# braincorp/bc-gym-planning-env

Hardware: AMD Instinct MI355X
Metric: env-steps/sec at N=65536 RandomMiniEnv, 1/2/4/8 MI355X; % HBM roofline (higher is better)
Workload: dtype f64

## Files before the change

bc_gym_planning_env_amd/csrc/bcp_step.h:

```cpp
#pragma once

#include <hip/hip_runtime.h>

#include <cstddef>
#include <cstdint>
#include <type_traits>

#include "bcp_device.h"
#include "bcp_raster.h"
#include "bcp_coop.h"

using namespace bcp;

struct DevState {
    double *x, *y, *angle, *v, *w, *steer, *wheel, *min_dist;
    int32_t *target_idx, *cur_iter;
    uint8_t* collided;
    double *pose_seen, *state_seen;
    double *control_q, *pose_q, *state_q;
};

struct MapDesc {
    const uint32_t* bits;
    const uint32_t* tiles;
// ... 630 lines not shown
{
    if (delay <= 0) return;
    const int slot = (k - 1) % delay;
    double* cell = q + ((int64_t)slot * W) * n + i;
    if (k <= delay) {
#pragma unroll
        for (int c = 0; c < W; ++c) cell[c * n] = v[c];
        if (k > 1) {
#pragma unroll
            for (int c = 0; c < W; ++c) v[c] = q[c * n + i];
        }
    } else {
#pragma unroll
        for (int c = 0; c < W; ++c) {
            const double first = cell[c * n];
            cell[c * n] = v[c];
            v[c] = first;
        }
    }
}

template <int W>
__device__ __forceinline__ void fifo_peek(const double* __restrict__ q, int delay, int64_t n, int64_t i, int k, double (&peeked)[W])
{
    if (delay <= 0 || k <= 1) return;
    const double* cell = q + ((int64_t)(k > delay ? (k - 1) % delay : 0) * W) * n + i;
#pragma unroll
    for (int c = 0; c < W; ++c) peeked[c] = cell[c * n];
}

template <int W>
__device__ __forceinline__ void fifo_push(double* __restrict__ q, int delay, int64_t n, int64_t i, int k, double (&v)[W],
                                          const double (&peeked)[W])
{
    if (delay <= 0) return;
    double* cell = q + ((int64_t)((k - 1) % delay) * W) * n + i;
#pragma unroll
    for (int c = 0; c < W; ++c) {
        cell[c * n] = v[c];
        if (k > 1) v[c] = peeked[c];
    }
}

constexpr int kWavePerPoseFrom = 1;
#ifdef BCP_DIAG
constexpr int kDiagBlocks = 4096;
__device__ unsigned long long g_diag[kDiagBlocks * 16];
#define DIAG_STAMP(k) do { if (threadIdx.x == 0 && blockIdx.x < 512) g_diag[blockIdx.x * 16 + (k)] = __builtin_amdgcn_s_memtime(); } while (0)
#define DIAG_STAMP_W(w, k) do { if (threadIdx.x == (w) * 64 && blockIdx.x < kDiagBlocks) g_diag[blockIdx.x * 16 + (k)] = __builtin_amdgcn_s_memtime(); } while (0)
#define DIAG_MAX(k, v) do { if ((threadIdx.x & 63) == 0 && blockIdx.x < 2048) atomicMax(&g_diag[(2048 + blockIdx.x) * 16 + (k)], (unsigned long long)(v)); } while (0)
#define DIAG_NOW() __builtin_amdgcn_s_memtime()
#define DIAG_REAL_ENTRY() do { if ((threadIdx.x & 63) == 0 && blockIdx.x < 1024) atomicMax(&g_diag[(3072 + blockIdx.x) * 16 + 0], ~(unsigned long long)__builtin_amdgcn_s_memrealtime()); } while (0)
#define DIAG_REAL_EXIT() do { if ((threadIdx.x & 63) == 0 && blockIdx.x < 1024) atomicMax(&g_diag[(3072 + blockIdx.x) * 16 + 1], (unsigned long long)__builtin_amdgcn_s_memrealtime()); } while (0)
#define DIAG_STAMP_U(w, k) do { if (threadIdx.x == (w) * 64 && blockIdx.x < 2048) g_diag[(2048 + blockIdx.x) * 16 + (k)] = __builtin_amdgcn_s_memtime(); } while (0)
#define DIAG_WAIT_VMEM() asm volatile("s_waitcnt vmcnt(0)" ::: "memory")
#define DIAG_STAMP_WAVES(base) do { if ((threadIdx.x & 63) == 0 && blockIdx.x < 256) g_diag[((base) + blockIdx.x) * 16 + (threadIdx.x >> 6)] = __builtin_amdgcn_s_memtime(); } while (0)
#define DIAG_MAX_ALL(k, v) do { if (blockIdx.x < 2048) atomicMax(&g_diag[(2048 + blockIdx.x) * 16 + (k)], (unsigned long long)(v)); } while (0)
extern "C" int bcp_diag_read(unsigned long long* out)
{
    return (int)hipMemcpyFromSymbol(out, HIP_SYMBOL(g_diag), sizeof(g_diag));
}
extern "C" int bcp_diag_clear()
{
    void* p = nullptr;
    if (hipGetSymbolAddress(&p, HIP_SYMBOL(g_diag)) != hipSuccess) return -1;
    return (int)hipMemset(p, 0, sizeof(g_diag));
}

#else
#define DIAG_STAMP(k) do { } while (0)
#define DIAG_STAMP_W(w, k) do { } while (0)
#define DIAG_MAX(k, v) do { } while (0)
#define DIAG_NOW() 0ull
#define DIAG_REAL_ENTRY() do { } while (0)
#define DIAG_REAL_EXIT() do { } while (0)
#define DIAG_STAMP_U(w, k) do { } while (0)
#define DIAG_WAIT_VMEM() do { } while (0)
#define DIAG_STAMP_WAVES(base) do { } while (0)
#define DIAG_MAX_ALL(k, v) do { } while (0)
#endif


extern __shared__ uint32_t lds_dyn[];

struct CollisionLds {
    bool staged;
    LdsWords bits;
    LdsF64 qverts;
    VertLds scratch;
    LdsU32 cells;
};

__device__ __forceinline__ CollisionLds collision_lds_setup(const DevParams& P, const MapDesc& map, int tid)
{
    CollisionLds L;
    const int map_words = map.in_lds ? map.rows * map.wpr : 0;
    const LdsU32 lds = (LdsU32)lds_dyn;
    for (int k = tid; k < map_words; k += kBlock) lds[k] = map.bits[k];
    const int q_off = (map_words + 1) & ~1;
    __attribute__((address_space(3))) double* q = (__attribute__((address_space(3))) double*)(lds + q_off);
    for (int k = tid; k < 2 * P.n_verts; k += kBlock) q[k] = P.qverts[k >> 1][k & 1];
    L.staged = map.in_lds != 0;
    L.bits = lds;
    L.qverts = q;
    L.scratch.base = lds + q_off + 4 * P.n_verts + tid;
    L.scratch.stride = kBlock;
    L.cells = lds + q_off + 4 * P.n_verts + 2 * P.n_verts * kBlock;
    __syncthreads();
    return L;
}

static size_t collision_lds_bytes(int n_verts, int in_lds, int rows, int wpr)
{
    size_t words = in_lds ? (size_t)rows * wpr : 0;
    words = (words + 1) & ~(size_t)1;
    words += 4 * (size_t)n_verts;
    words += 2 * (size_t)n_verts * kBlock;
    words += kSparseLdsWords;
    return words * sizeof(uint32_t);
}

__device__ __forceinline__ bool collides_wave(const DevParams& P, const MapDesc& map, const CullDesc& cull,
                                              const CollisionLds& L, int exact_mode, int dense_threshold, bool wide,
                                              bool active, int64_t env, double x, double y, double th)
{
    double ox = map.ox, oy = map.oy;
    if (map.origins) {
        ox = map.origins[2 * env + 0];
// ... 39 lines not shown
            else
                verdict = wide ? coop_collides_sparse<true>(P, L.qverts, c_, s_, px_, py_, words, map.rows, map.cols, map.wpr, L.cells)
                               : coop_collides_sparse<false>(P, L.qverts, c_, s_, px_, py_, words, map.rows, map.cols, map.wpr, L.cells);
        }
        if (verdict != kSparseTooMany) {
            h = verdict == kSparseHit;
        } else if (L.staged) {
            h = coop_collides(P, vqx, vqy, c_, s_, px_, py_, L.bits, map.rows, map.cols, map.wpr, wide);
        } else {
            h = coop_collides(P, vqx, vqy, c_, s_, px_, py_, words, map.rows, map.cols, map.wpr, wide);
        }
        if (lane_id() == src) hit = h;
    }
    return hit;
}

struct Pending {
    double c, s;
    int32_t px, py;
    Robot r;
    Pose old;
    double min_dist;
    double z[3];
    int32_t target, iter, err, drawn;
    int32_t collided;
    int32_t env_lo, env_hi;
    int32_t geom;
    double popped_pose[3], popped_state[7];
};

struct InitAhead {
    double x, y, th, v, w, steer, wheel, min_dist;
    int32_t target, iter, collided;
};

template <typename SP>
__device__ __forceinline__ InitAhead fetch_init_ahead(SP S, int64_t k, bool tri)
{
    InitAhead p;
    p.x = as_global(S->init.x)[k];
    p.y = as_global(S->init.y)[k];
    p.th = as_global(S->init.angle)[k];
    p.v = as_global(S->init.v)[k];
    p.w = as_global(S->init.w)[k];
    p.steer = tri ? as_global(S->init.steer)[k] : 0.0;
    p.wheel = tri ? as_global(S->init.wheel)[k] : 0.0;
    p.min_dist = as_global(S->init.min_dist)[k];
    p.target = as_global(S->init.target_idx)[k];
    p.iter = as_global(S->init.cur_iter)[k];
    p.collided = (int32_t)as_global(S->init.collided)[k];
    return p;
}

struct ScoredFree {
    double rew, min_dist;
    int target;
};

struct ParkedPose {
    double c, s;
    int32_t px, py;
    int32_t env_lo, env_hi;
    int32_t geom;
    int32_t verdict;
    double spec_rew, spec_min;
    int32_t spec_target, spec_ok;
};

template <typename SP>
__device__ __forceinline__ int64_t slot_of(SP S, int64_t i, const Pending& q)
{
    return S->geom_of_env ? (int64_t)q.geom : i;
}

template <bool PLAIN, typename A, typename SP>
__device__ __forceinline__ int finalize_env_from(const A& a, SP S, int64_t i, Pending& q, bool hit, LdsF64 lds_path = nullptr,
                                             const PathWindow* free_window = nullptr, bool have_score = false,
                                             ScoredFree score = ScoredFree(), int known_len = -1, bool score_fits_hit = false,
                                             int64_t out_base = 0, RecRedo redo = RecRedo{0.0, -1, false})
{
    const DevParams& P = *(const DevParams*)&S->P;
    const int pose_delay = PLAIN ? 0 : P.pose_delay, state_delay = PLAIN ? 0 : P.state_delay;
    const bool pure_pursuit = !PLAIN && P.reward_provider == BCP_REWARD_PURE_PURSUIT;
    const bool tri = P.model == BCP_MODEL_TRICYCLE;
    const int64_t n = S->n;
    Robot& r = q.r;
    if (hit) {
        r.p = q.old;
        r.v = 0.0;
        r.w = 0.0;
    }
    int iter = q.iter + 1;
    bool collided = q.collided != 0 || hit;
    double min_dist = q.min_dist;
    int target = q.target;
    double seen[3] = {r.p.x, r.p.y, r.p.th};
    double seen_rs[7] = {r.p.x, r.p.y, r.p.th, r.v, r.w, r.steer, r.wheel};
    if (pose_delay) fifo_push<3>(S->st.pose_q, pose_delay, n, i, iter, seen, q.popped_pose);
    if (state_delay) fifo_push<7>(S->st.state_q, state_delay, n, i, iter, seen_rs, q.popped_state);

    double rew = 0.0;
    int m;
    bool goal;
    const int64_t g = slot_of(S, i, q);
    const double* pts = S->path.pts + (S->path.shared ? 0 : g * (int64_t)S->path.max_len * 5);
    m = known_len >= 0 ? known_len : (S->path.shared ? S->path.max_len : S->path.lens[g]);
    if (pure_pursuit) {
        if (have_score && !hit) {
            rew = score.rew;
            min_dist = score.min_dist;
            target = score.target;
        } else if (!ABLATED(a, kAblateNoReward)) {
            rew = reward_pure_pursuit(pts, m, seen[0], seen[1], collided, min_dist, target);
        }
        goal = hypot(pts[5 * (m - 1)] - seen[0], pts[5 * (m - 1) + 1] - seen[1]) < 1.0;
    } else {
        if (have_score && (!hit || score_fits_hit || (pose_delay && iter > 1))) {
            rew = score.rew;
            min_dist = score.min_dist;
            target = score.target;
        } else if (!ABLATED(a, kAblateNoReward)) {
            const PathWindow w =
                (free_window && !hit && !pose_delay) ? *free_window : path_window_of(P, S->path.shared != 0, S->path.bbox, S->path.index, g, seen[0], seen[1]);
            if (lds_path && S->path.shared)
                rew = reward_step(P, lds_path, w, m, seen[0], seen[1], seen[2], min_dist, target);
            else
                rew = reward_step<PLAIN ? 4 : 2>(P, pts, w, m, seen[0], seen[1], seen[2], min_dist, target);
        }
        goal = target > m - 1;
    }
    const bool timeout = iter >= P.iteration_timeout;
    const bool done = goal || timeout || collided;

    const int64_t o = out_base + i;
    as_global(a.reward)[o] = rew;
    as_global(a.done)[o] = (uint8_t)done;
    if (a.collided_now) as_global(a.collided_now)[o] = (uint8_t)hit;
    if (a.err) as_global(a.err)[o] = q.err;
    if (a.noise_z_out) {
        const double nan = __builtin_nan("");
        as_global(a.noise_z_out)[3 * o + 0] = (q.drawn & 1) ? q.z[0] : nan;
        as_global(a.noise_z_out)[3 * o + 1] = (q.drawn & 2) ? q.z[1] : nan;
        as_global(a.noise_z_out)[3 * o + 2] = (q.drawn & 4) ? q.z[2] : nan;
    }

    const bool reset = done && (a.flags & BCP_STEP_AUTO_RESET);
    InitAhead ahead = InitAhead();
    if (reset) {
        int64_t k = i;
        if (S->geom_of_env) {
            k = S->next_geom ? as_global(S->next_geom)[g] : g;
            as_global(S->geom_of_env)[i] = (int32_t)k;
        }
        ahead = fetch_init_ahead(S, k, tri);
    }
    int rec_slot = -1;
    if (a.flags & kStepRecord) {
        const EpisodeRec& R = a.S->rec;
        double ret_sum = 0.0;
        if (R.ret) ret_sum = (redo.on ? redo.ret_before : as_global(R.ret)[i]) + rew;
        as_global(R.reason)[i] = done ? (uint8_t)((goal ? BCP_DONE_GOAL : 0) | (timeout ? BCP_DONE_TIMEOUT : 0) |
                                                  (collided ? BCP_DONE_COLLIDED : 0))
                                      : (uint8_t)0;
        const bool keeps = redo.on && redo.slot >= 0;
        const bool take = done && !keeps;
        const uint64_t takers = __ballot(take);
        if (takers) {
            const int first = (int)__ffsll((unsigned long long)takers) - 1;
            const int lane = lane_id();
            int base = 0;
            if (lane == first) base = (int)atomicAdd(R.work, (uint32_t)__popcll(takers));
            base = bcast_i(base, first);
            if (take) rec_slot = base + (int)__popcll(takers & ((1ull << lane) - 1ull));
        }
        if (keeps) rec_slot = redo.slot;
        if (done && rec_slot < R.capacity) {
            const int64_t j = rec_slot, c = R.capacity;
            as_global(R.env_id)[j] = (int32_t)i;
            as_global(R.geom)[j] = S->geom_of_env ? (int32_t)g : -1;
            if (R.ret) as_global(R.final_ret)[j] = ret_sum;
            as_global(R.fin.x)[j] = r.p.x;
            as_global(R.fin.y)[j] = r.p.y;
            as_global(R.fin.angle)[j] = r.p.th;
            as_global(R.fin.v)[j] = r.v;
            as_global(R.fin.w)[j] = r.w;
            if (tri) {
                as_global(R.fin.steer)[j] = r.steer;
                as_global(R.fin.wheel)[j] = r.wheel;
            }
            as_global(R.fin.min_dist)[j] = min_dist;
            as_global(R.fin.target_idx)[j] = target;
            as_global(R.fin.cur_iter)[j] = iter;
            as_global(R.fin.collided)[j] = (uint8_t)collided;
            if (pose_delay) {
#pragma unroll
                for (int k = 0; k < 3; ++k) R.fin.pose_seen[k * c + j] = seen[k];
            }
            if (state_delay) {
#pragma unroll
                for (int k = 0; k < 7; ++k) R.fin.state_seen[k * c + j] = seen_rs[k];
            }
        }
        if (!done) rec_slot = -1;
        if (R.ret) as_global(R.ret)[i] = reset ? 0.0 : ret_sum;
    }
    if (reset) {
        r.p.x = ahead.x;
// ... 355 lines not shown
                Pending q = *e;
                finalize_env<PLAIN>(a, i, q, true, nullptr, nullptr, false, ScoredFree(), -1, false,
                                    redo_of(a, (int64_t)idx * kShards + shard));
            }
        }
        if (a.flags & kStepRecord) {
            __syncthreads();
            if (threadIdx.x == 0) record_publish(a.S, gridDim.x);
        }
        return;
    }
    for (int idx = blockIdx.x / kShards; idx < a.hot.pending_cap; idx += stride) {
        const Pending* e = slots + (int64_t)idx * kShards;
        const double c = e->c, s = e->s;
        const int px = e->px, py = e->py;
        const int64_t i = ((int64_t)e->env_hi << 32) | (uint32_t)e->env_lo;
        const int64_t g = a.hot.geom_of_env ? (int64_t)e->geom : i;
        if (idx >= count) break;
        DIAG_STAMP(1);
        const uint32_t* words = a.hot.map_bits + (a.hot.map_shared ? 0 : g * a.hot.map_env_stride);
        bool hit = false;
        DIAG_STAMP(2);
        if (!ABLATED(a, kAblateNoCoop))
            hit = coop_collides_quad<WIDE>(P, vqx, vqy, c, s, px, py, words, a.hot.map_rows, a.hot.map_cols, a.hot.map_wpr, wave,
                                           (LdsU32)lds_dyn);
        DIAG_STAMP(3);
        hit = __syncthreads_or(hit);
        DIAG_STAMP(4);
        if (hit && threadIdx.x == 0) {
            Pending q = *e;
            finalize_env<PLAIN>(a, i, q, true, nullptr, nullptr, false, ScoredFree(), -1, false,
                                redo_of(a, (int64_t)idx * kShards + shard));
        }
    }
    if (a.flags & kStepRecord) {
        __syncthreads();
        if (threadIdx.x == 0) record_publish(a.S, gridDim.x);
    }
}


constexpr int kLocalPairsMax = 4;
constexpr int kLocalPairsDefault = 4;

typedef const __attribute__((address_space(4))) StepArgs& KernArgs;

constexpr int kScanItems = 1024;
constexpr int kHandDoubles = 8;
constexpr int kLocalMapWords = 4096;

typedef uint32_t u32x4 __attribute__((ext_vector_type(4)));
constexpr int kStaticChunks = (int)((offsetof(StepStatic, rec) + 15) / 16);

static size_t local_step_lds_bytes(int n_verts, int lds_path_doubles, int staged_map_words, bool plain = true, int pairs = kLocalPairsMax)
{
    const int kLocalPairs = pairs, kLocalWaves = 4 * pairs, kLocalEnvs = pairs * kBlock;
    size_t bytes = ((size_t)2 * n_verts + lds_path_doubles + (size_t)kLocalPairs * kHandDoubles * kBlock + 8) * sizeof(double);
    bytes += 2 * kBlock * sizeof(uint32_t);
    bytes += 16 * sizeof(int32_t);
    bytes = (bytes + 15) & ~(size_t)15;
    bytes += (size_t)kLocalEnvs * sizeof(ParkedPose);
    bytes += (size_t)kLocalWaves * kSparseLdsWords * sizeof(uint32_t);
    bytes += (size_t)staged_map_words * sizeof(uint32_t);
    bytes = (bytes + 15) & ~(size_t)15;
    bytes += kStaticChunks * 16;
    if (!plain) bytes += (size_t)10 * kLocalEnvs * sizeof(double);
    return bytes;
}

template <int NW>
__device__ __forceinline__ void fetch_words(const __attribute__((address_space(4))) void* p, uint32_t (&w)[NW])
{
    const __attribute__((address_space(4))) uint32_t* src = (const __attribute__((address_space(4))) uint32_t*)p;
#pragma unroll
    for (int k = 0; k < NW; ++k) w[k] = src[k];
}

template <int NW>
__device__ __forceinline__ void pin_words(uint32_t (&w)[NW])
{
#pragma unroll
    for (int k = 0; k < NW; ++k) {
        asm("" : "+s"(w[k]));
        w[k] = (uint32_t)__builtin_amdgcn_readfirstlane((int)w[k]);
    }
}

struct PrologueArgs {
    StepHot hot;
    const StepStatic* S;
    const void* actions;
    const double* noise_z;
    uint64_t* tick;
    uint32_t flags;
};

__device__ __forceinline__ uint64_t uniform_u64(uint64_t v)
{
    const uint32_t lo = (uint32_t)__builtin_amdgcn_readfirstlane((int)(uint32_t)v);
    const uint32_t hi = (uint32_t)__builtin_amdgcn_readfirstlane((int)(uint32_t)(v >> 32));
    return ((uint64_t)hi << 32) | lo;
}

static_assert(kStaticChunks <= 128, "*S is staged by the last two waves of a workgroup");
constexpr int kPollLimit = 1 << 16;
#define BOUNDED_POLL(cond, expired) do { int trips_ = 0; while (cond) { __builtin_amdgcn_s_sleep(1); if (++trips_ > kPollLimit) { (expired) = true; break; } } } while (0)
constexpr uint32_t kDiagWithholdVerdicts = 1u << 23;

typedef const __attribute__((address_space(4))) StepArgs* KernArgPtr;

template <bool WIDE, bool PLAIN, int PAIRS, bool ROLL>
__device__ __forceinline__ void step_local_body(KernArgPtr kernarg, const int rs)
{
    static_assert(PAIRS == 1 || PAIRS == 2 || PAIRS == 4, "a workgroup holds 1, 2 or 4 (mover, scorer, helper, helper) quartets");
    constexpr int kLocalPairs = PAIRS, kLocalWaves = 4 * PAIRS, kLocalEnvs = PAIRS * kBlock;
    constexpr int kPairShift = PAIRS == 4 ? 2 : (PAIRS == 2 ? 1 : 0);
    constexpr int kStaticFrom = (kLocalWaves - 2) * kBlock;
    constexpr int kCtlFrom = (kLocalWaves - 1) * kBlock;
    [[maybe_unused]] constexpr int kWScorer = PAIRS, kWHelper1 = 2 * PAIRS, kWHelper2 = 3 * PAIRS;
    DIAG_STAMP_WAVES(512);
    DIAG_REAL_ENTRY();
    const int tid = threadIdx.x, lane = tid & 63, wave = tid >> 6;
    const bool mover = wave < kLocalPairs, scorer = wave >= kLocalPairs && wave < 2 * kLocalPairs;
    const int pair = wave & (kLocalPairs - 1);
    KernArgs a = *kernarg;
    PrologueArgs L;
    {
        constexpr int kStateWords = PLAIN ? kHotStateWords : (int)(sizeof(DevState) / 4);
        uint32_t w_st[kStateWords], w_hot[kHotPrologueWords];
        fetch_words(&a.hot.st, w_st);
        fetch_words(&a.hot.n, w_hot);
        pin_words(w_st);
        pin_words(w_hot);
        __builtin_memset(&L.hot, 0, sizeof(L.hot));
        __builtin_memcpy(&L.hot.st, w_st, sizeof(w_st));
        __builtin_memcpy(&L.hot.n, w_hot, sizeof(w_hot));
        L.actions = L.hot.io_actions;
        L.noise_z = L.hot.io_noise_z;
        L.tick = L.hot.io_tick;
        L.flags = L.hot.io_flags;
        L.S = a.S;
        if (ROLL) {
            const int64_t row = (int64_t)rs * L.hot.n;
            L.actions = (const char*)L.actions + row * ((L.flags & BCP_STEP_ACTIONS_F32) ? 8 : 16);
            L.noise_z = L.noise_z ? L.noise_z + 3 * row : nullptr;
        }
    }
    const int64_t out_base = ROLL ? (int64_t)rs * L.hot.n : 0;
    const int hot_n_verts = L.hot.n_verts, hot_npath = L.hot.lds_path_doubles, hot_path_shared = L.hot.path_shared;
    const int hot_map_rows = L.hot.map_rows, hot_map_cols = L.hot.map_cols, hot_map_wpr = L.hot.map_wpr;
    const int hot_map_shared = L.hot.map_shared, hot_noise_on = L.hot.noise_on, hot_max_len = L.hot.path_max_len;
    const int64_t hot_n = L.hot.n;
    const bool scanner = PLAIN ? !mover : scorer;
    const int member = (wave >> kPairShift) - 1;

    __attribute__((address_space(3))) double* qv = (__attribute__((address_space(3))) double*)lds_dyn;
    const int nq = 2 * hot_n_verts;
    const int npath = hot_npath;
    const LdsF64 lds_path = npath ? (LdsF64)(qv + nq) : (LdsF64) nullptr;
    __attribute__((address_space(3))) double* hand_pose = qv + nq + npath + pair * kHandDoubles * kBlock;
    __attribute__((address_space(3))) double* hand_score = hand_pose + 3 * kBlock;
    __attribute__((address_space(3))) double* hand_heading = hand_pose + 6 * kBlock;
    __attribute__((address_space(3))) double* lds_box = qv + nq + npath + kLocalPairs * kHandDoubles * kBlock;
    __attribute__((address_space(3))) uint32_t* lds_index = (__attribute__((address_space(3))) uint32_t*)(lds_box + 8);
    __attribute__((address_space(3))) int32_t* ctl = (__attribute__((address_space(3))) int32_t*)(lds_index + 2 * kBlock);
    const uint32_t rec_off = (uint32_t)((((size_t)(nq + npath + kLocalPairs * kHandDoubles * kBlock + 8) * sizeof(double) +
                                          2 * kBlock * sizeof(uint32_t) + 16 * sizeof(int32_t)) + 15) & ~(size_t)15);
    __attribute__((address_space(3))) ParkedPose* rec =
        (__attribute__((address_space(3))) ParkedPose*)((__attribute__((address_space(3))) char*)lds_dyn + rec_off);
    const LdsU32 cell_list = (LdsU32)(rec + kLocalEnvs) + wave * kSparseLdsWords;
    const LdsU32 lds_map = (LdsU32)(rec + kLocalEnvs) + kLocalWaves * kSparseLdsWords;
    const int map_words = ((hot_map_shared != 0) & (hot_map_rows * hot_map_wpr <= kLocalMapWords)) ? hot_map_rows * hot_map_wpr : 0;
    const uint32_t static_off = (uint32_t)(((size_t)((__attribute__((address_space(3))) char*)(lds_map + map_words) -
                                                     (__attribute__((address_space(3))) char*)lds_dyn) + 15) & ~(size_t)15);
    __attribute__((address_space(3))) u32x4* lds_static = (__attribute__((address_space(3))) u32x4*)((__attribute__((address_space(3))) char*)lds_dyn + static_off);
    const __attribute__((address_space(3))) StepStatic* SL = (const __attribute__((address_space(3))) StepStatic*)lds_static;
    __attribute__((address_space(3))) double* fifo_stash = (__attribute__((address_space(3))) double*)(lds_static + kStaticChunks) + pair * kBlock + lane;

    DIAG_STAMP(0);
    DIAG_STAMP_WAVES(768);
    const int64_t gi = (int64_t)blockIdx.x * kLocalEnvs + pair * kBlock + lane;
    const bool active = gi < hot_n;
    const int64_t i = active ? gi : hot_n - 1;
    const bool noise_by_waves = (hot_noise_on != 0) & (L.noise_z == nullptr);

    uint64_t tick_counter = 0, tick_seed = 0;
    if (!mover) {
        int zero;
        asm("v_mov_b32 %0, 0" : "=v"(zero));
        const GlobalPtr<const uint64_t> t = as_global((const uint64_t*)L.tick) + zero;
        tick_counter = t[0];
        tick_seed = t[2];
    }
    Pending q;
    double cmd0 = 0.0, cmd1 = 0.0;
    float box[8] = {0, 0, 0, 0, 0, 0, 0, 0};
    float quant_inv = 0.0f;
    double old_angle = 0.0;
    double own_org_x = 0.0, own_org_y = 0.0;
    uint64_t own_len_shift = 0;
    const bool own_origin = !hot_path_shared || L.hot.map_origins != nullptr;
    if (mover) {
        load_env<PLAIN>(L, 0, 0, i, active, q, cmd0, cmd1, false);
        if (!hot_path_shared) {
            const int64_t g = L.hot.geom_of_env ? (int64_t)q.geom : i;
            own_org_x = as_global(L.hot.path_bbox)[g * kBoxDoubles + kBoxOrigin];
            own_org_y = as_global(L.hot.path_bbox)[g * kBoxDoubles + kBoxOrigin + 1];
            own_len_shift = as_global(reinterpret_cast<const uint64_t*>(L.hot.path_bbox))[g * kBoxDoubles + kBoxLenWord / 2];
        } else if (L.hot.map_origins) {
            const int64_t g = L.hot.geom_of_env ? (int64_t)q.geom : i;
            own_org_x = as_global(L.hot.map_origins)[2 * g + 0];
            own_org_y = as_global(L.hot.map_origins)[2 * g + 1];
        }
    } else {
        if (scanner) {
            if (!PLAIN) q.min_dist = as_global(L.hot.st.min_dist)[i];
            q.target = as_global(L.hot.st.target_idx)[i];
            q.geom = L.hot.geom_of_env ? as_global(L.hot.geom_of_env)[i] : 0;
            q.collided = PLAIN ? 0 : (int32_t)(as_global(L.hot.st.collided)[i] != 0);
            if (!hot_path_shared) {
                const int64_t g = L.hot.geom_of_env ? (int64_t)q.geom : i;
#pragma unroll
                for (int k = 0; k < 8; ++k) box[k] = as_global(reinterpret_cast<const float*>(L.hot.path_bbox + g * kBoxDoubles))[k];
                quant_inv = as_global(reinterpret_cast<const float*>(L.hot.path_bbox + g * kBoxDoubles))[kBoxQuantStep + 1];
                own_len_shift = as_global(reinterpret_cast<const uint64_t*>(L.hot.path_bbox))[g * kBoxDoubles + kBoxLenWord / 2];
            }
        }
        if (member == 1) old_angle = as_global(L.hot.st.angle)[i];
    }
    double rc[9] = {0, 0, 0, 0, 0, 0, 0, 0, 0};
    if (PLAIN && mover) {
// ... 57 lines not shown
    }
    if (tid >= kCtlFrom && tid < kCtlFrom + 16) ctl[tid - kCtlFrom] = 0;
    if (first_trip && tid >= kStaticFrom && tid < kStaticFrom + kStaticChunks) lds_static[tid - kStaticFrom] = st_static;
    DIAG_STAMP_WAVES(1024);
    __syncthreads();
    const DevParams& P = *(const DevParams*)&SL->P;
    const int map_rows = hot_map_rows, map_cols = hot_map_cols;
    const int my_len = hot_path_shared ? hot_max_len : (int)(uint32_t)own_len_shift;
    Pose new_pose;
    new_pose.x = new_pose.y = new_pose.th = 0.0;
    if (mover) {
        if (noise_by_waves) {
            q.z[0] = hand_score[lane];
            q.z[1] = hand_score[kBlock + lane];
            q.z[2] = hand_score[2 * kBlock + lane];
        }
        DIAG_STAMP(1);
        if (!PLAIN) drive = robot_step_begin(P, r, cmd0, cmd1);
        new_pose = robot_step_pose(P, r, drive, q.z, q.drawn);
        const bool delayed = !PLAIN && P.pose_delay > 0 && q.iter + 1 > 1;
        hand_pose[lane] = delayed ? fifo_stash[0] : new_pose.x;
        hand_pose[kBlock + lane] = delayed ? fifo_stash[kLocalEnvs] : new_pose.y;
        hand_pose[2 * kBlock + lane] = delayed ? fifo_stash[2 * kLocalEnvs] : new_pose.th;
        DIAG_STAMP(2);
    }
    if (!mover && member == 1) {
        double c0, s0;
        cos_sin(old_angle, c0, s0);
        hand_heading[lane] = c0;
        hand_heading[kBlock + lane] = s0;
        DIAG_STAMP_U(kWHelper1, 2);
    }
    if (!mover && first_trip) {
        constexpr int kStagers = (kLocalWaves - kLocalPairs) * kBlock;
        constexpr int kMapPerStager = (kLocalMapWords + kStagers - 1) / kStagers;
        constexpr int kBoxAt = kStagers >= 448 ? 256 : kStagers - 8;
        constexpr int kIndexAt = kStagers >= 448 ? 320 : kStagers - 136;
        const int nm = tid - kLocalPairs * kBlock;
        double st_q = 0.0, st_path = 0.0;
        float st_box = 0.0f;
        uint32_t st_index = 0;
        uint32_t st_map[kMapPerStager] = {};
        if (nm < nq) st_q = as_global(L.hot.qverts)[nm];
        if (nm < npath) st_path = as_global(L.hot.path_pts)[nm];
        if (hot_path_shared) {
            if (nm >= kBoxAt && nm < kBoxAt + 8) st_box = as_global(reinterpret_cast<const float*>(L.hot.path_bbox))[nm - kBoxAt];
            if (nm >= kIndexAt && nm < kIndexAt + 128) st_index = as_global(reinterpret_cast<const uint32_t*>(L.hot.path_index))[nm - kIndexAt];
        }
#pragma unroll
        for (int u = 0; u < kMapPerStager; ++u) {
            const int k = u * kStagers + nm;
            if (k < map_words) st_map[u] = as_global(L.hot.map_bits)[k];
        }
        if (nm < nq) qv[nm] = st_q;
        if (nm < npath) qv[nq + nm] = st_path;
        for (int k = kStagers + nm; k < npath; k += kStagers) qv[nq + k] = as_global(L.hot.path_pts)[k];
        if (hot_path_shared) {
            if (nm >= kBoxAt && nm < kBoxAt + 8) lds_box[nm - kBoxAt] = (double)st_box;
            if (nm >= kIndexAt && nm < kIndexAt + 128) lds_index[nm - kIndexAt] = st_index;
        }
#pragma unroll
        for (int u = 0; u < kMapPerStager; ++u) {
            const int k = u * kStagers + nm;
            if (k < map_words) lds_map[k] = st_map[u];
        }
    }
    DIAG_STAMP_WAVES(1536);
    __syncthreads();
    DIAG_STAMP(3);
    if (mover) {
        KnownHeading old_heading;
        old_heading.c0 = hand_heading[lane];
        old_heading.s0 = hand_heading[kBlock + lane];
        old_heading.known = true;
        q.err = robot_step_measure(P, r, new_pose, old_heading);
    }
    bool park = false;
    bool poll_expired = false;
    if (mover) {
        OuterParams outer = outer_params(*(const CullDesc*)&SL->cull);
        outer.near_tx = SL->cull.step_near_tx;
        outer.near_shift = SL->cull.step_near_shift;
        const double map_inv_res = SL->map.inv_res;
        const int64_t near_stride = SL->cull.step_near_stride;
        const double org_x = own_origin ? own_org_x : SL->map.ox, org_y = own_origin ? own_org_y : SL->map.oy;
        const int64_t g = slot_of(SL, i, q);
        const int px = (int)rint((r.p.x - org_x) * map_inv_res);
        const int py = (int)rint((r.p.y - org_y) * map_inv_res);
        double c, s;
        cos_sin(r.p.th, c, s);
        DIAG_STAMP_U(0, 4);
        const int64_t map_env = a.hot.map_shared ? 0 : g;
        int cls = kFree;
#ifdef BCP_DIAG
        if (!ABLATED(a, kAblateNoCollision | kAblateNoClassify))
#endif
        {
            if (a.hot.near) {
                cls = classify_near(outer, as_global(a.hot.near) + map_env * near_stride, map_rows, map_cols, px, py, c, s);
            } else {
                const OuterLookups look = outer_lookups_issue(*(const CullDesc*)&SL->cull, map_env, map_rows, map_cols, px, py, c, s);
                cls = outer_lookups_verdict(*(const CullDesc*)&SL->cull, look);
            }
        }
        if (!active) cls = kFree;
        DIAG_STAMP_U(0, 5);
        if (cls == kAmbiguous && !ABLATED(a, kAblateNoPark)) {
            park = true;
            q.c = c;
            q.s = s;
            q.px = px;
            q.py = py;
            q.env_lo = (int32_t)(uint32_t)i;
            q.env_hi = (int32_t)(i >> 32);
        }
    } else if (scanner && !ABLATED(a, kAblateNoReward)) {
        const double x = hand_pose[lane], y = hand_pose[kBlock + lane], th = hand_pose[2 * kBlock + lane];
// ... 179 lines not shown
    DIAG_STAMP_W(kWHelper1, 9);
    const double vqx = lane < P.n_verts ? qv[2 * lane] : 0.0, vqy = lane < P.n_verts ? qv[2 * lane + 1] : 0.0;
    DIAG_STAMP(7);
    __attribute__((address_space(3))) int* const ticket_word =
        lane == 0 ? (__attribute__((address_space(3))) int*)&ctl[1] : (__attribute__((address_space(3))) int*)(cell_list + lane);
    int ticket = __builtin_amdgcn_readfirstlane(__hip_atomic_fetch_add(ticket_word, lane == 0 ? 1 : 0, __ATOMIC_RELAXED, __HIP_MEMORY_SCOPE_WORKGROUP));
    while (ticket < n_parked) {
        DIAG_STAMP_W(kWHelper1, 10);
        __attribute__((address_space(3))) ParkedPose* e = rec + ticket;
        const double c = e->c, s = e->s;
        const int px = e->px, py = e->py;
        const int64_t env = ((int64_t)e->env_hi << 32) | (uint32_t)e->env_lo;
        const int64_t g = a.hot.map_shared ? 0 : (a.hot.geom_of_env ? (int64_t)e->geom : env);
        const uint32_t* words = a.hot.map_bits + g * a.hot.map_env_stride;
        const uint32_t* tiles = a.map_tiles + g * map_tile_words(a.hot.map_rows, a.hot.map_wpr);
        bool h = false;
        [[maybe_unused]] const unsigned long long test_from = DIAG_NOW();
        [[maybe_unused]] int how = 0;
        if (!ABLATED(a, kAblateNoCoop)) {
#ifdef BCP_DIAG
            unsigned long long phase[3] = {test_from, test_from, 0};
            unsigned long long* const phases = phase;
#else
            unsigned long long* const phases = nullptr;
#endif
            const int verdict = map_words
                ? coop_collides_sparse<WIDE>(P, (LdsF64)qv, c, s, px, py, (LdsWords)lds_map, a.hot.map_rows, a.hot.map_cols,
                                             a.hot.map_wpr, cell_list, phases)
                : coop_collides_sparse<WIDE, true>(P, (LdsF64)qv, c, s, px, py, as_global(tiles), a.hot.map_rows, a.hot.map_cols,
                                                   a.hot.map_wpr, cell_list, phases);
#ifdef BCP_DIAG
            if (threadIdx.x == kWHelper1 * 64 && blockIdx.x < 2048) {
                const unsigned long long now = DIAG_NOW();
                g_diag[(2048 + blockIdx.x) * 16 + 13] = ((phase[0] - test_from) << 40) | ((phase[1] - phase[0]) << 20) | (now - phase[1]);
                g_diag[(2048 + blockIdx.x) * 16 + 15] = phase[2];
            }
#endif
            h = verdict == kSparseHit;
            if (verdict == kSparseTooMany)
                h = coop_collides<WIDE>(P, vqx, vqy, c, s, px, py, words, a.hot.map_rows, a.hot.map_cols, a.hot.map_wpr);
            how = verdict;
        }
        DIAG_MAX(0, ((DIAG_NOW() - test_from) << 4) | (unsigned)how);
        DIAG_STAMP_W(kWHelper1, 11);
        bool post = lane == 0;
#ifdef BCP_DIAG
        post = post && !(a.flags & kDiagWithholdVerdicts);
#endif
        if (post) __hip_atomic_store(&e->verdict, h ? 2 : 1, __ATOMIC_RELEASE, __HIP_MEMORY_SCOPE_WORKGROUP);
        ticket = __builtin_amdgcn_readfirstlane(__hip_atomic_fetch_add(ticket_word, lane == 0 ? 1 : 0, __ATOMIC_RELAXED, __HIP_MEMORY_SCOPE_WORKGROUP));
        DIAG_STAMP_W(kWHelper1, 12);
    }
    if (mover) {
        int verdict = park ? 0 : 1;
        {
            int trips = 0;
            while (__ballot(verdict == 0)) {
                if (verdict == 0) verdict = __hip_atomic_load(&my_rec->verdict, __ATOMIC_ACQUIRE, __HIP_MEMORY_SCOPE_WORKGROUP);
                __builtin_amdgcn_s_sleep(1);
                if (++trips > kPollLimit) {
                    poll_expired = true;
                    if (verdict == 0) {
                        verdict = 1;
                        q.err |= BCP_ERR_INTERNAL;
                    }
                    break;
                }
            }
        }
        const bool hit_score = PLAIN && lds_path && a.hot.path_shared && !ABLATED(a, kAblateNoReward);
        int last_hit = -1;
        if (hit_score) {
            uint64_t hits = __ballot(park && verdict == 2);
            while (hits) {
                const int src = (int)__ffsll((unsigned long long)hits) - 1;
                hits &= hits - 1;
                const double ox = bcast_d(q.old.x, src), oy = bcast_d(q.old.y, src), oth = bcast_d(q.old.th, src);
                const int tg = bcast_i(q.target, src);
                const PathWindow w = path_window(P, (LdsF64)lds_box, (const __attribute__((address_space(3))) int16_t*)lds_index, ox, oy);
                const int found = coop_last_reached(P, lds_path, w, my_len, tg, ox, oy, oth);
                if (lane == src) last_hit = found;
            }
        }
        if (active) {
            const bool hit_now = park && verdict == 2;
            bool fits = hit_score && hit_now;
            if (fits) {
                sc.min_dist = q.min_dist;
                sc.target = q.target;
                sc.rew = reward_from_last(P, lds_path, my_len, last_hit, q.old.x, q.old.y, sc.min_dist, sc.target);
            } else if (PLAIN && hit_now && my_rec->spec_ok) {
                sc.rew = my_rec->spec_rew;
                sc.min_dist = my_rec->spec_min;
                sc.target = my_rec->spec_target;
                fits = true;
            }
            if (!PLAIN) {
#pragma unroll
                for (int k = 0; k < 3; ++k) q.popped_pose[k] = fifo_stash[k * kLocalEnvs];
#pragma unroll
                for (int k = 0; k < 7; ++k) q.popped_state[k] = fifo_stash[(3 + k) * kLocalEnvs];
            }
            finalize_env_from<PLAIN>(a, SL, i, q, hit_now, lds_path, nullptr, !ABLATED(a, kAblateNoReward), sc, my_len, fits, out_base);
        }
        if ((a.flags & kStepRecord) && lane == 0 &&
            __hip_atomic_fetch_add(&ctl[3], 1, __ATOMIC_ACQ_REL, __HIP_MEMORY_SCOPE_WORKGROUP) == kLocalPairs - 1) {
            __threadfence();
            unsigned int* ticket = reinterpret_cast<unsigned int*>(a.tick + kTickLocalTicket);
            if (atomicAdd(ticket, 1u) == gridDim.x - 1) {
                *ticket = 0u;
                a.tick[0] = a.tick[0] + 1;
                record_store_count(a.S->rec);
            }
        }
    }
    DIAG_STAMP(13);
    DIAG_STAMP_W(kWHelper1, 14);
#ifdef BCP_DIAG
    if (tid == 0 && blockIdx.x < kDiagBlocks) g_diag[blockIdx.x * 16 + 15] = (unsigned long long)n_parked;
#endif
    if (poll_expired && lane == 0) atomicAdd(reinterpret_cast<unsigned long long*>(a.tick + 4), 1ull);
    DIAG_REAL_EXIT();
    if ((a.flags & kStepAdvances) && tid == (kLocalWaves - 1) * kBlock) {
        if (n_parked) a.parked_slots[blockIdx.x] += (uint64_t)n_parked;
        if ((!ROLL || rs == a.rollout_steps - 1) && !(a.flags & kStepRecord)) {
            const unsigned int ticket_drawn =
                __hip_atomic_fetch_add((GlobalPtr<unsigned int>)(a.tick + kTickLocalTicket), 1u, __ATOMIC_RELAXED, __HIP_MEMORY_SCOPE_AGENT);
            if (ticket_drawn == gridDim.x - 1) {
                *reinterpret_cast<unsigned int*>(a.tick + kTickLocalTicket) = 0u;
                a.tick[0] = step_counter + 1;
            }
        }
    }
}

template <bool WIDE, bool PLAIN, int PAIRS>
__device__ __attribute__((noinline)) void step_local_trip(uint64_t kernarg_bits, int rs)
{
    const uint32_t lo = (uint32_t)__builtin_amdgcn_readfirstlane((int)(uint32_t)kernarg_bits);
    const uint32_t hi = (uint32_t)__builtin_amdgcn_readfirstlane((int)(uint32_t)(kernarg_bits >> 32));
    step_local_body<WIDE, PLAIN, PAIRS, true>((KernArgPtr)(uintptr_t)(((uint64_t)hi << 32) | lo), __builtin_amdgcn_readfirstlane(rs));
}

template <bool WIDE, bool PLAIN, int PAIRS, bool ROLL = false>
__global__ void __attribute__((amdgpu_flat_work_group_size(4 * PAIRS * kBlock, 4 * PAIRS * kBlock), amdgpu_waves_per_eu(4)))
step_local_kernel(const StepArgs launch_args)
{
    KernArgPtr kernarg = (KernArgPtr)__builtin_amdgcn_kernarg_segment_ptr();
    if constexpr (!ROLL) {
        step_local_body<WIDE, PLAIN, PAIRS, false>(kernarg, 0);
    } else {
        const int n_steps = kernarg->rollout_steps;
        for (int rs = 0; rs < n_steps; ++rs) {
            step_local_trip<WIDE, PLAIN, PAIRS>((uint64_t)(uintptr_t)kernarg, rs);
            __syncthreads();
        }
    }
// ... 2 lines not shown
```

bc_gym_planning_env_amd/csrc/bcp_step_host.h:

```cpp
#pragma once

static bool step_is_plain(const bcp_handle* h)
{
    const bcp_params& p = h->params;
    return p.control_delay == 0 && p.pose_delay == 0 && p.state_delay == 0 && p.reward_provider == BCP_REWARD_CONTINUOUS;
}

static bool step_uses_deferral(const bcp_handle* h)
{
    return h->defer && h->cull.on && h->exact_mode == 0 && h->pending.get() != nullptr;
}

static int step_form(const bcp_handle* h)
{
    if (!step_uses_deferral(h)) return 0;
    if (h->dense_threshold < 0) return 1;
    return (h->fused && h->adaptive) ? 3 : 2;
}

static int upload_step_static(bcp_handle* h, hipStream_t s)
{
    StepStatic& S = h->host_static;
    S.P = h->dev;
    S.map = h->map;
// ... 92 lines not shown
        default: return BCP_LOCAL_FN(false, false);
    }
#undef BCP_LOCAL_FN
}

static int local_pairs(const bcp_handle* h)
{
    if (h->local_pairs == 1 || h->local_pairs == 2 || h->local_pairs == 4) return h->local_pairs;
    return kLocalPairsDefault;
}

static int launch_step(bcp_handle* h, const bcp_step_io* io, uint32_t flags, hipStream_t s, bool first_only = false,
                       int32_t rollout_steps = 1)
{
    if (h->static_dirty) BCP_TRY(upload_step_static(h, s));
    const StepStatic& S = h->host_static;
    const int form = step_form(h);
    const bool fused = form == 3;
    if (!fused && h->edt_lazy) BCP_TRY(ensure_fields(h, s));
    if ((form == 1 || form == 2) && (h->last_step_form == 0 || h->last_step_form == 3)) BCP_TRY(rearm_parking(h, s));
    h->last_step_form = form;
    StepArgs a;
    a.S = h->dev_static.get();
    a.hot = h->host_hot;
    a.actions = io->actions;
    a.noise_z = io->noise_z;
    a.noise_z_out = io->noise_z_out;
    a.reward = io->reward;
    a.done = io->done;
    a.collided_now = io->collided_now;
    a.err = io->err;
    a.flags = flags;
    if (h->have_rec) a.flags |= kStepRecord;
    a.seed = a.step_counter = 0;
    a.pending_count = a.pending_next = nullptr;
    a.threshold_now = nullptr;
    a.threshold_next = a.inplace_count = a.inplace_next = nullptr;
    const bool adapt = h->adaptive && h->adapt.get() && S.pending && S.dense_threshold >= 0;
    a.tick = h->tick.get();
    a.parked_slots = nullptr;
    a.map_tiles = S.map.tiles;
    a.rollout_steps = 1;
    a.pending_base = h->pending_count.get();
    a.adapt_base = adapt ? h->adapt.get() : nullptr;
    const int blocks = (int)((h->n + kBlock - 1) / kBlock);
    const int variant = (S.wide ? 2 : 0) | (step_is_plain(h) ? 1 : 0);
    if (fused) {
        const bool roll = rollout_steps > 1;
        const int pairs = roll ? 4 : local_pairs(h);
        a.rollout_steps = rollout_steps;
        const int64_t bitmap_words = (int64_t)S.map.rows * S.map.wpr;
        const size_t lds = local_step_lds_bytes(h->params.n_verts, S.lds_path_doubles,
                                                (S.map.shared && bitmap_words <= kLocalMapWords) ? (int)bitmap_words : 0,
                                                step_is_plain(h), pairs);
        a.flags |= kStepAdvances;
        a.hot.io_flags = a.flags;
        a.hot.io_actions = a.actions;
        a.hot.io_noise_z = a.noise_z;
        a.hot.io_tick = a.tick;
        const int envs_per_group = pairs * kBlock;
        const dim3 grid((unsigned)((h->n + envs_per_group - 1) / envs_per_group)), block(4 * pairs * kBlock);
        if (!h->parked_slots.get()) {
            HIP_TRY(h->parked_slots.reserve((size_t)((h->n + kBlock - 1) / kBlock)));
            HIP_TRY(hipMemsetAsync(h->parked_slots.get(), 0, h->parked_slots.capacity() * sizeof(uint64_t), s));
        }
        a.parked_slots = h->parked_slots.get();
        return launch_variant(h, local_step_fn(variant, pairs, roll), grid, block, lds, s, a);
    }
    if (rollout_steps > 1) return fail(BCP_E_STATE, "launch_step: only the single-launch step form takes several steps per launch");
    if (form == 0) {
        const size_t lds = collision_lds_bytes(h->params.n_verts, h->map.in_lds, h->map.rows, h->map.wpr);
        a.flags |= kStepAdvances;
        hipLaunchKernelGGL(step_kernel, dim3(blocks), dim3(kBlock), lds, s, a);
        return BCP_OK;
    }
    const size_t lds1 = ((size_t)h->params.n_verts * 2 + S.lds_path_doubles) * sizeof(double);
    const size_t lds2 = (size_t)2 * 4 * (S.wide ? 8 : 3) * 64 * sizeof(uint32_t);
    const int waves = 2048;
    const bool second = !first_only && S.dense_threshold >= 0;
    if (!second) a.flags |= kStepAdvances;
    const size_t lds1p = lds1 + ((size_t)6 * kBlock + 8) * sizeof(double) + 2 * kBlock * sizeof(uint32_t);
    const int rc = launch_variant(h, kFastPairFn[variant], dim3(blocks), dim3(2 * kBlock), lds1p, s, a);
    if (rc != BCP_OK || !second) return rc;
    return launch_variant(h, kPendingFn[variant], dim3(waves), dim3(kBlock * kPendingWaves), lds2, s, a);
}

#ifdef BCP_DIAG
constexpr uint32_t kCallerFlags = BCP_STEP_AUTO_RESET | BCP_STEP_ACTIONS_F32 | kAblateNoCollision | kAblateNoReward |
                                  kAblateNoCoop | kAblateNoPark | kAblateNoClassify | kDiagWithholdVerdicts;
#else
constexpr uint32_t kCallerFlags = BCP_STEP_AUTO_RESET | BCP_STEP_ACTIONS_F32;
#endif

static int check_step(bcp_handle* h, const bcp_step_io* io, uint32_t flags, const char* who)
{
    if (!h || !io) return fail(BCP_E_INVALID, "%s: null argument", who);
    if (flags & ~kCallerFlags) return fail(BCP_E_INVALID, "%s: undefined flag bits 0x%x", who, flags & ~kCallerFlags);
    if (!h->have_map || !h->have_path || !h->have_state)
        return fail(BCP_E_STATE, "%s: costmaps, paths and state must be set first", who);
    if ((flags & BCP_STEP_AUTO_RESET) && !h->have_init)
        return fail(BCP_E_STATE, "%s: BCP_STEP_AUTO_RESET needs bcp_bind_initial_state", who);
    if (!io->actions || !io->reward || !io->done) return fail(BCP_E_INVALID, "%s: actions/reward/done are required", who);
    return BCP_OK;
}

constexpr uint32_t kWatchdogSteps = 256;

// ... 282 lines not shown
```

Baseline: 5.802 billion.

## Overlap hit-rescoring with verdict polling and stage reset init state in LDS

Moves the cooperative last-reached path scan and reward rescoring for parked poses inside the verdict-polling loop, so the scoring runs while waves would otherwise sleep waiting for collision verdicts. Prefetches per-env reset init state into LDS during the staging phase for plain, non-geometry runs, so auto-reset reads LDS instead of scattered global loads in the tail. Packs the output pointers into a compact TailArgs fetched as words. This costs extra LDS per pair, which may reduce occupancy, and the staging loads run even for envs that never reset. It also adds diagnostic tail stamps that compile away by default.

```diff
diff --git a/bc_gym_planning_env_amd/csrc/bcp_step.h b/bc_gym_planning_env_amd/csrc/bcp_step.h
--- a/bc_gym_planning_env_amd/csrc/bcp_step.h
+++ b/bc_gym_planning_env_amd/csrc/bcp_step.h
@@ -706,6 +706,8 @@
 #define DIAG_NOW() __builtin_amdgcn_s_memtime()
 #define DIAG_REAL_ENTRY() do { if ((threadIdx.x & 63) == 0 && blockIdx.x < 1024) atomicMax(&g_diag[(3072 + blockIdx.x) * 16 + 0], ~(unsigned long long)__builtin_amdgcn_s_memrealtime()); } while (0)
 #define DIAG_REAL_EXIT() do { if ((threadIdx.x & 63) == 0 && blockIdx.x < 1024) atomicMax(&g_diag[(3072 + blockIdx.x) * 16 + 1], (unsigned long long)__builtin_amdgcn_s_memrealtime()); } while (0)
+#define DIAG_TAIL_MAX(k, v) do { if (blockIdx.x < 1024) atomicMax(&g_diag[(3072 + blockIdx.x) * 16 + (k)], (unsigned long long)(v)); } while (0)
+#define DIAG_TAIL_STAMP(k) do { if ((threadIdx.x & 63) == 0) DIAG_TAIL_MAX(k, __builtin_amdgcn_s_memtime()); } while (0)
 #define DIAG_STAMP_U(w, k) do { if (threadIdx.x == (w) * 64 && blockIdx.x < 2048) g_diag[(2048 + blockIdx.x) * 16 + (k)] = __builtin_amdgcn_s_memtime(); } while (0)
 #define DIAG_WAIT_VMEM() asm volatile("s_waitcnt vmcnt(0)" ::: "memory")
 #define DIAG_STAMP_WAVES(base) do { if ((threadIdx.x & 63) == 0 && blockIdx.x < 256) g_diag[((base) + blockIdx.x) * 16 + (threadIdx.x >> 6)] = __builtin_amdgcn_s_memtime(); } while (0)
@@ -728,6 +730,8 @@
 #define DIAG_NOW() 0ull
 #define DIAG_REAL_ENTRY() do { } while (0)
 #define DIAG_REAL_EXIT() do { } while (0)
+#define DIAG_TAIL_MAX(k, v) do { } while (0)
+#define DIAG_TAIL_STAMP(k) do { } while (0)
 #define DIAG_STAMP_U(w, k) do { } while (0)
 #define DIAG_WAIT_VMEM() do { } while (0)
 #define DIAG_STAMP_WAVES(base) do { } while (0)
@@ -873,6 +877,28 @@
     return p;
 }
 
+constexpr int kInitLdsBytes = (8 * 8 + 2 * 4 + 1) * kBlock;
+typedef const __attribute__((address_space(3))) char* LdsInit;
+
+__device__ __forceinline__ InitAhead read_init_ahead(LdsInit block, int lane, bool tri)
+{
+    const __attribute__((address_space(3))) double* d = (const __attribute__((address_space(3))) double*)block + lane;
+    const __attribute__((address_space(3))) int32_t* w = (const __attribute__((address_space(3))) int32_t*)(block + 8 * 8 * kBlock) + lane;
+    InitAhead p;
+    p.x = d[0];
+    p.y = d[kBlock];
+    p.th = d[2 * kBlock];
+    p.v = d[3 * kBlock];
+    p.w = d[4 * kBlock];
+    p.steer = tri ? d[5 * kBlock] : 0.0;
+    p.wheel = tri ? d[6 * kBlock] : 0.0;
+    p.min_dist = d[7 * kBlock];
+    p.target = w[0];
+    p.iter = w[kBlock];
+    p.collided = (int32_t)((const __attribute__((address_space(3))) uint8_t*)(block + (8 * 8 + 2 * 4) * kBlock))[lane];
+    return p;
+}
+
 struct ScoredFree {
     double rew, min_dist;
     int target;
@@ -898,7 +924,7 @@
 __device__ __forceinline__ int finalize_env_from(const A& a, SP S, int64_t i, Pending& q, bool hit, LdsF64 lds_path = nullptr,
                                              const PathWindow* free_window = nullptr, bool have_score = false,
                                              ScoredFree score = ScoredFree(), int known_len = -1, bool score_fits_hit = false,
-                                             int64_t out_base = 0, RecRedo redo = RecRedo{0.0, -1, false})
+                                             int64_t out_base = 0, RecRedo redo = RecRedo{0.0, -1, false}, LdsInit init_lds = nullptr)
 {
     const DevParams& P = *(const DevParams*)&S->P;
     const int pose_delay = PLAIN ? 0 : P.pose_delay, state_delay = PLAIN ? 0 : P.state_delay;
@@ -966,6 +992,7 @@
     }
 
     const bool reset = done && (a.flags & BCP_STEP_AUTO_RESET);
+    if (reset || hit) DIAG_TAIL_MAX(2, hit ? 2 : 1);
     InitAhead ahead = InitAhead();
     if (reset) {
         int64_t k = i;
@@ -973,7 +1000,7 @@
             k = S->next_geom ? as_global(S->next_geom)[g] : g;
             as_global(S->geom_of_env)[i] = (int32_t)k;
         }
-        ahead = fetch_init_ahead(S, k, tri);
+        ahead = init_lds ? read_init_ahead(init_lds, lane_id(), tri) : fetch_init_ahead(S, k, tri);
     }
     int rec_slot = -1;
     if (a.flags & kStepRecord) {
@@ -1435,7 +1462,8 @@
 typedef uint32_t u32x4 __attribute__((ext_vector_type(4)));
 constexpr int kStaticChunks = (int)((offsetof(StepStatic, rec) + 15) / 16);
 
-static size_t local_step_lds_bytes(int n_verts, int lds_path_doubles, int staged_map_words, bool plain = true, int pairs = kLocalPairsMax)
+static size_t local_step_lds_bytes(int n_verts, int lds_path_doubles, int staged_map_words, bool plain = true, int pairs = kLocalPairsMax,
+                                   bool init_staged = false)
 {
     const int kLocalPairs = pairs, kLocalWaves = 4 * pairs, kLocalEnvs = pairs * kBlock;
     size_t bytes = ((size_t)2 * n_verts + lds_path_doubles + (size_t)kLocalPairs * kHandDoubles * kBlock + 8) * sizeof(double);
@@ -1448,6 +1476,7 @@
     bytes = (bytes + 15) & ~(size_t)15;
     bytes += kStaticChunks * 16;
     if (!plain) bytes += (size_t)10 * kLocalEnvs * sizeof(double);
+    if (plain && init_staged) bytes += (size_t)kLocalPairs * kInitLdsBytes;
     return bytes;
 }
 
@@ -1477,6 +1506,21 @@
     uint64_t* tick;
     uint32_t flags;
 };
+
+struct TailArgs {
+    const __attribute__((address_space(4))) StepHot& hot;
+    const StepStatic* S;
+    double* noise_z_out;
+    double* reward;
+    uint8_t* done;
+    uint8_t* collided_now;
+    int32_t* err;
+    uint32_t flags;
+};
+constexpr int kTailWords = 5 * 2;
+static_assert(offsetof(StepArgs, err) + 8 - offsetof(StepArgs, noise_z_out) == kTailWords * 4 &&
+              offsetof(StepArgs, reward) == offsetof(StepArgs, noise_z_out) + 8 && offsetof(StepArgs, done) == offsetof(StepArgs, reward) + 8 &&
+              offsetof(StepArgs, collided_now) == offsetof(StepArgs, done) + 8, "the output pointers of StepArgs are adjacent");
 
 __device__ __forceinline__ uint64_t uniform_u64(uint64_t v)
 {
@@ -1560,6 +1604,9 @@
     const __attribute__((address_space(3))) StepStatic* SL = (const __attribute__((address_space(3))) StepStatic*)lds_static;
     __attribute__((address_space(3))) double* fifo_stash = (__attribute__((address_space(3))) double*)(lds_static + kStaticChunks) + pair * kBlock + lane;
 
+    const bool stage_init = PLAIN && !L.hot.geom_of_env && (L.flags & BCP_STEP_AUTO_RESET);
+    __attribute__((address_space(3))) char* const init_block = (__attribute__((address_space(3))) char*)(lds_static + kStaticChunks) + pair * kInitLdsBytes;
+
     DIAG_STAMP(0);
     DIAG_STAMP_WAVES(768);
     const int64_t gi = (int64_t)blockIdx.x * kLocalEnvs + pair * kBlock + lane;
@@ -1723,6 +1770,28 @@
             const int k = u * kStagers + nm;
             if (k < map_words) st_map[u] = as_global(L.hot.map_bits)[k];
         }
+        double st_init[4] = {0.0, 0.0, 0.0, 0.0};
+        int32_t st_init_w[2] = {0, 0};
+        uint8_t st_init_b = 0;
+        const bool staging_init = stage_init && active;
+        if (staging_init) {
+            const bool tri = L.hot.model == BCP_MODEL_TRICYCLE;
+            if (member == 0) {
+                st_init[0] = as_global(SL->init.x)[gi];
+                st_init[1] = as_global(SL->init.y)[gi];
+                st_init[2] = as_global(SL->init.angle)[gi];
+                st_init[3] = as_global(SL->init.v)[gi];
+            } else if (member == 1) {
+                st_init[0] = as_global(SL->init.w)[gi];
+                if (tri) st_init[1] = as_global(SL->init.steer)[gi];
+                if (tri) st_init[2] = as_global(SL->init.wheel)[gi];
+                st_init[3] = as_global(SL->init.min_dist)[gi];
+            } else {
+                st_init_w[0] = as_global(SL->init.target_idx)[gi];
+                st_init_w[1] = as_global(SL->init.cur_iter)[gi];
+                st_init_b = as_global(SL->init.collided)[gi];
+            }
+        }
         if (nm < nq) qv[nm] = st_q;
         if (nm < npath) qv[nq + nm] = st_path;
         for (int k = kStagers + nm; k < npath; k += kStagers) qv[nq + k] = as_global(L.hot.path_pts)[k];
@@ -1734,6 +1803,18 @@
         for (int u = 0; u < kMapPerStager; ++u) {
             const int k = u * kStagers + nm;
             if (k < map_words) lds_map[k] = st_map[u];
+        }
+        if (staging_init) {
+            if (member < 2) {
+                __attribute__((address_space(3))) double* d = (__attribute__((address_space(3))) double*)init_block + member * 4 * kBlock + lane;
+#pragma unroll
+                for (int k = 0; k < 4; ++k) d[k * kBlock] = st_init[k];
+            } else {
+                __attribute__((address_space(3))) int32_t* w = (__attribute__((address_space(3))) int32_t*)(init_block + 8 * 8 * kBlock) + lane;
+                w[0] = st_init_w[0];
+                w[kBlock] = st_init_w[1];
+                ((__attribute__((address_space(3))) uint8_t*)(init_block + (8 * 8 + 2 * 4) * kBlock))[lane] = st_init_b;
+            }
         }
     }
     DIAG_STAMP_WAVES(1536);
@@ -2019,11 +2100,45 @@
         DIAG_STAMP_W(kWHelper1, 12);
     }
     if (mover) {
+        uint32_t w_tail[kTailWords];
+        fetch_words(&a.noise_z_out, w_tail);
+        pin_words(w_tail);
+        const auto tail_ptr = [&w_tail](int k) { return (void*)(uintptr_t)(((uint64_t)w_tail[2 * k + 1] << 32) | w_tail[2 * k]); };
+        const TailArgs T = {a.hot, L.S, (double*)tail_ptr(0), (double*)tail_ptr(1), (uint8_t*)tail_ptr(2), (uint8_t*)tail_ptr(3),
+                            (int32_t*)tail_ptr(4), L.flags};
+        const bool hit_score = PLAIN && lds_path && a.hot.path_shared && !ABLATED(a, kAblateNoReward);
         int verdict = park ? 0 : 1;
+        uint64_t unscanned = hit_score ? __ballot(park) : 0ull;
+        int last_hit = -1;
+        bool old_scored = false;
+        ScoredFree old = sc;
         {
             int trips = 0;
-            while (__ballot(verdict == 0)) {
+            for (;;) {
                 if (verdict == 0) verdict = __hip_atomic_load(&my_rec->verdict, __ATOMIC_ACQUIRE, __HIP_MEMORY_SCOPE_WORKGROUP);
+                const bool waiting = __ballot(verdict == 0) != 0ull;
+                const bool wanted = park && (waiting || verdict == 2);
+                const uint64_t need = hit_score ? __ballot(wanted) : 0ull;
+                if (need & unscanned) {
+                    const int src = (int)__ffsll((unsigned long long)(need & unscanned)) - 1;
+                    unscanned &= ~(1ull << src);
+                    const double ox = bcast_d(q.old.x, src), oy = bcast_d(q.old.y, src), oth = bcast_d(q.old.th, src);
+                    const int tg = bcast_i(q.target, src);
+                    const PathWindow w = path_window(P, (LdsF64)lds_box, (const __attribute__((address_space(3))) int16_t*)lds_index, ox, oy);
+                    const int found = coop_last_reached(P, lds_path, w, my_len, tg, ox, oy, oth);
+                    if (lane == src) last_hit = found;
+                    continue;
+                }
+                if (need && !old_scored) {
+                    if (wanted) {
+                        old.min_dist = q.min_dist;
+                        old.target = q.target;
+                        old.rew = reward_from_last(P, lds_path, my_len, last_hit, q.old.x, q.old.y, old.min_dist, old.target);
+                    }
+                    old_scored = true;
+                    continue;
+                }
+                if (!waiting) break;
                 __builtin_amdgcn_s_sleep(1);
                 if (++trips > kPollLimit) {
                     poll_expired = true;
@@ -2031,31 +2146,15 @@
                         verdict = 1;
                         q.err |= BCP_ERR_INTERNAL;
                     }
-                    break;
                 }
             }
         }
-        const bool hit_score = PLAIN && lds_path && a.hot.path_shared && !ABLATED(a, kAblateNoReward);
-        int last_hit = -1;
-        if (hit_score) {
-            uint64_t hits = __ballot(park && verdict == 2);
-            while (hits) {
-                const int src = (int)__ffsll((unsigned long long)hits) - 1;
-                hits &= hits - 1;
-                const double ox = bcast_d(q.old.x, src), oy = bcast_d(q.old.y, src), oth = bcast_d(q.old.th, src);
-                const int tg = bcast_i(q.target, src);
-                const PathWindow w = path_window(P, (LdsF64)lds_box, (const __attribute__((address_space(3))) int16_t*)lds_index, ox, oy);
-                const int found = coop_last_reached(P, lds_path, w, my_len, tg, ox, oy, oth);
-                if (lane == src) last_hit = found;
-            }
-        }
+        DIAG_TAIL_STAMP(4);
         if (active) {
             const bool hit_now = park && verdict == 2;
             bool fits = hit_score && hit_now;
             if (fits) {
-                sc.min_dist = q.min_dist;
-                sc.target = q.target;
-                sc.rew = reward_from_last(P, lds_path, my_len, last_hit, q.old.x, q.old.y, sc.min_dist, sc.target);
+                sc = old;
             } else if (PLAIN && hit_now && my_rec->spec_ok) {
                 sc.rew = my_rec->spec_rew;
                 sc.min_dist = my_rec->spec_min;
@@ -2068,8 +2167,10 @@
 #pragma unroll
                 for (int k = 0; k < 7; ++k) q.popped_state[k] = fifo_stash[(3 + k) * kLocalEnvs];
             }
-            finalize_env_from<PLAIN>(a, SL, i, q, hit_now, lds_path, nullptr, !ABLATED(a, kAblateNoReward), sc, my_len, fits, out_base);
-        }
+            finalize_env_from<PLAIN>(T, SL, i, q, hit_now, lds_path, nullptr, !ABLATED(a, kAblateNoReward), sc, my_len, fits, out_base,
+                                     RecRedo{0.0, -1, false}, stage_init ? (LdsInit)init_block : (LdsInit) nullptr);
+        }
+        DIAG_TAIL_STAMP(3);
         if ((a.flags & kStepRecord) && lane == 0 &&
             __hip_atomic_fetch_add(&ctl[3], 1, __ATOMIC_ACQ_REL, __HIP_MEMORY_SCOPE_WORKGROUP) == kLocalPairs - 1) {
             __threadfence();
diff --git a/bc_gym_planning_env_amd/csrc/bcp_step_host.h b/bc_gym_planning_env_amd/csrc/bcp_step_host.h
--- a/bc_gym_planning_env_amd/csrc/bcp_step_host.h
+++ b/bc_gym_planning_env_amd/csrc/bcp_step_host.h
@@ -168,7 +168,7 @@
         const int64_t bitmap_words = (int64_t)S.map.rows * S.map.wpr;
         const size_t lds = local_step_lds_bytes(h->params.n_verts, S.lds_path_doubles,
                                                 (S.map.shared && bitmap_words <= kLocalMapWords) ? (int)bitmap_words : 0,
-                                                step_is_plain(h), pairs);
+                                                step_is_plain(h), pairs, S.geom_of_env == nullptr);
         a.flags |= kStepAdvances;
         a.hot.io_flags = a.flags;
         a.hot.io_actions = a.actions;
```

New measurement: 5.485 billion. 0.945x the previous value.
